# twesterhout/distributed-matvec

Hardware: AMD Instinct MI355X
Metric: matvecs/sec (higher is better)
Workload: dtype f64; 1 GPU; heisenberg_chain_32: y <- H x, 601080390 basis states, 9927521280 off-diagonal non-zeros, f64 vectors, sigma/x/y resident in HBM; partitions=1, partitioning=single, exchange=none, kernel=direct-pull+staged, x=u(hash(sigma, 42)) - 0.5, exchange_bytes_per_matvec=0

## Files before the change

### distributed-matvec_amd/_lib.py

```python
from __future__ import annotations

import ctypes as C
import os

_HERE = os.path.dirname(os.path.abspath(__file__))
LIB_PATH = os.path.join(_HERE, os.environ.get("LS_AMD_LIB", "libls_amd.so"))

c_u64p = C.POINTER(C.c_uint64)
c_i64p = C.POINTER(C.c_int64)
c_f64p = C.POINTER(C.c_double)
c_intp = C.POINTER(C.c_int)


class ChplExternalArray(C.Structure):

    _fields_ = [("elts", C.c_void_p), ("num_elts", C.c_uint64), ("freer", C.c_void_p)]


class LsHsBasis(C.Structure):

    _fields_ = [
        ("number_sites", C.c_int),
        ("number_particles", C.c_int),
        ("number_up", C.c_int),
# ... 72 lines not shown
        "ls_amd_device_count": (C.c_int, []),
        "ls_amd_set_device": (C.c_int, [C.c_int]),
        "ls_amd_malloc": (C.c_int, [C.POINTER(vp), C.c_size_t]),
        "ls_amd_free": (C.c_int, [vp]),
        "ls_amd_memcpy_h2d": (C.c_int, [vp, vp, C.c_size_t]),
        "ls_amd_memcpy_d2h": (C.c_int, [vp, vp, C.c_size_t]),
        "ls_amd_memcpy_d2d": (C.c_int, [vp, vp, C.c_size_t, vp]),
        "ls_amd_memset": (C.c_int, [vp, C.c_int, C.c_size_t, vp]),
        "ls_amd_synchronize": (C.c_int, [vp]),
        "ls_amd_stream_copy": (C.c_int, [vp, vp, C.c_int64, vp]),
        "ls_amd_stream_read": (C.c_int, [vp, C.c_int64, C.c_int, vp, vp]),
        "ls_amd_orth_max_rows": (C.c_int, []),
        "ls_amd_orth_pass": (C.c_int, [C.c_int, C.c_int64, vp, C.c_int64, vp, vp, vp, vp]),
        "ls_amd_basis_rotate": (C.c_int, [C.c_int, C.c_int, C.c_int64, vp, C.c_int64, vp, vp]),
        "ls_amd_orth_block_max_rows": (C.c_int, []),
        "ls_amd_orth_block_pass": (C.c_int, [C.c_int, C.c_int, C.c_int64, vp, C.c_int64, vp, C.c_int64, vp, vp, vp]),
        "ls_amd_block_rotate": (C.c_int, [C.c_int, C.c_int, C.c_int64, vp, C.c_int64, vp, vp]),
        "ls_amd_pointer_kind": (C.c_int, [vp]),
        "ls_amd_host_register": (C.c_int, [vp, C.c_size_t]),
        "ls_amd_host_unregister": (C.c_int, [vp]),
        "ls_amd_boundary_stats_get": (None, [C.POINTER(BoundaryStats), C.c_int]),
        "ls_amd_hash64_01": (C.c_uint64, [C.c_uint64]),
        "ls_amd_locale_idx_of": (C.c_int, [C.c_uint64, C.c_int]),
        "ls_amd_plan_create": (C.c_int, [C.POINTER(vp), op, C.c_int, C.c_int, C.c_int, C.POINTER(vp), c_i64p, C.c_int, C.c_int, vp]),
        "ls_amd_plan_create_replicated": (C.c_int, [C.POINTER(vp), op, C.c_int, C.c_int, C.c_int, vp, C.c_int64, vp, C.c_int64, vp]),
        "ls_amd_matvec_replicated": (C.c_int, [vp, vp, vp, vp]),
        "ls_amd_plan_destroy": (None, [vp]),
        "ls_amd_plan_num_rounds": (C.c_int, [vp]),
        "ls_amd_plan_kernel_name": (C.c_char_p, [vp]),
        "ls_amd_plan_send_counts": (C.c_int, [vp, C.c_int, c_i64p]),
        "ls_amd_plan_packet_bytes": (C.c_int, [vp]),
        "ls_amd_plan_row_bytes": (C.c_int, [vp]),
        "ls_amd_plan_nnz": (C.c_int64, [vp]),
        "ls_amd_plan_cache_slots": (C.c_int64, [vp, C.c_int64]),
        "ls_amd_plan_slot_cache_rows": (C.c_int, [vp, C.POINTER(C.c_int64), C.POINTER(C.c_int64)]),
        "ls_amd_matvec": (C.c_int, [vp, C.POINTER(vp), C.POINTER(vp), vp]),
        "ls_amd_matvec_block": (C.c_int, [vp, C.c_int, vp, C.c_int64, C.c_int64, vp, C.c_int64, C.c_int64, vp]),
        "ls_amd_plan_block_kernel_name": (C.c_char_p, [vp, C.c_int]),
        "ls_amd_matvec_block_axpby": (C.c_int, [vp, C.c_int, vp, C.c_int64, C.c_int64, vp, C.c_int64, C.c_int64, C.c_double, C.c_double,
                                                C.c_double, vp, vp]),
        "ls_amd_plan_axpby_kernel_name": (C.c_char_p, [vp, C.c_int]),
        "ls_amd_block_axpby_dots": (C.c_int, [C.c_int, C.c_int64, C.c_int, vp, C.c_int64, C.c_int64, vp, C.c_int64, C.c_int64, vp, C.c_int64,
                                              C.c_int64, C.c_double, C.c_double, C.c_double, vp, vp]),
        "ls_amd_matvec_block_axpby_acc": (C.c_int, [vp, C.c_int, vp, C.c_int64, C.c_int64, vp, C.c_int64, C.c_int64, C.c_double, C.c_double,
                                                    C.c_double, vp, C.c_int64, C.c_int64, C.c_int, C.c_double, C.c_double, vp, vp]),
        "ls_amd_plan_acc_kernel_name": (C.c_char_p, [vp, C.c_int]),
        "ls_amd_block_axpby_acc": (C.c_int, [C.c_int, C.c_int, C.c_int64, C.c_int, vp, C.c_int64, C.c_int64, vp, C.c_int64, C.c_int64, vp,
                                             C.c_int64, C.c_int64, vp, C.c_int64, C.c_int64, C.c_double, C.c_double, C.c_double, C.c_double,
                                             C.c_double, vp, vp]),
        "ls_amd_matvec_block_series": (C.c_int, [vp, C.c_int, C.c_int, vp, C.c_double, C.c_double, vp, C.c_int64, C.c_int64, vp, C.c_int64,
                                                 C.c_int64, C.c_int, vp, vp]),
        "ls_amd_plan_series_kernel_name": (C.c_char_p, [vp, C.c_int]),
        "ls_amd_plan_check": (C.c_int, [vp, vp]),
        "ls_amd_plan_enable_timing": (C.c_int, [vp, C.c_int]),
        "ls_amd_plan_kernel_times": (C.c_int, [vp, C.POINTER(C.c_float), C.c_int, c_intp]),
        "ls_amd_plan_enable_stage_timing": (C.c_int, [vp, C.c_int]),
        "ls_amd_plan_stage_times": (C.c_int, [vp, c_f64p, c_i64p, c_i64p]),
        "ls_amd_plan_timing_report": (C.c_int, [vp, C.c_char_p, C.c_size_t]),
        "ls_amd_operator_adjoint": (op, [op]),
        "ls_amd_operator_maps_sector": (C.c_int, [op, bp]),
        "ls_amd_operator_maps_sector_signed": (C.c_int, [op, bp]),
        "ls_amd_cross_create": (C.c_int, [C.POINTER(vp), op, bp, C.c_int, vp, C.c_int64, vp, C.c_int64, vp]),
        "ls_amd_operator_maps_subgroup_sector": (C.c_int, [op, bp]),
        "ls_amd_cross_create_groups": (C.c_int, [C.POINTER(vp), op, bp, C.c_int, C.c_int, vp, C.c_int64, vp, C.c_int64, vp]),
        "ls_amd_cross_apply": (C.c_int, [vp, vp, vp, vp]),
        "ls_amd_cross_apply_block": (C.c_int, [vp, C.c_int, vp, C.c_int64, C.c_int64, vp, C.c_int64, C.c_int64, vp]),
# ... 212 lines not shown
```

### distributed-matvec_amd/api.py

```python
from __future__ import annotations

import ctypes as C
from dataclasses import dataclass

import numpy as np

from . import _lib
from . import config as _config
from ._lib import LsAmdError

__all__ = [
    "Basis", "Operator", "LsAmdError", "loadConfigFromYaml", "loadConfigFromDict", "enumerateStates",
    "arrFromBlockToHashed", "arrFromHashedToBlock", "matrixVectorProduct", "localMatrixVector",
    "localeIdxOf", "hash64_01", "MatvecPlan", "ReplicatedPlan", "build_library", "fillRandom",
    "Communicator", "DistMatvec", "ReplMatvec", "block_axpby_dots", "block_axpby_acc", "CrossSectorPlan",
    "CsrMatrix",
]


def build_library(verbose: bool = False):
    import os
    import subprocess

    csrc = os.path.join(os.path.dirname(os.path.abspath(__file__)), "csrc")
# ... 461 lines not shown
        self.reps = reps
        self.P = num_partitions if num_partitions is not None else len(reps)
        self.me = my_partition
        self.cplx = dtype in (torch.complex128, "c128")
        n = len(reps)
        ptrs = (C.c_void_p * n)(*[r.data_ptr() for r in reps])
        counts = (C.c_int64 * n)(*[r.numel() for r in reps])
        h = C.c_void_p()
        _lib.check(L.ls_amd_plan_create(C.byref(h), matrix.payload, 1 if self.cplx else 0, self.P, my_partition,
                                        ptrs, counts, num_rounds, self.MODES[mode], _stream_ptr()))
        self.h = h

    def destroy(self):
        if getattr(self, "h", None):
            _lib.load().ls_amd_plan_destroy(self.h)
            self.h = None

    def __del__(self):
        try:
            self.destroy()
        except Exception:
            pass

    @property
    def kernel(self): return _lib.load().ls_amd_plan_kernel_name(self.h).decode()
    @property
    def num_rounds(self): return int(_lib.load().ls_amd_plan_num_rounds(self.h))
    @property
    def nnz(self): return int(_lib.load().ls_amd_plan_nnz(self.h))
    @property
    def packet_bytes(self): return int(_lib.load().ls_amd_plan_packet_bytes(self.h))
    @property
    def row_bytes(self): return int(_lib.load().ls_amd_plan_row_bytes(self.h))
    @property
    def key_bytes(self):
        return int(_lib.load().ls_amd_plan_key_bytes(self.h))
    @property
    def packet_index_bytes(self): return int(_lib.load().ls_amd_plan_packet_index_bytes(self.h))

    def segment_bytes(self, count: int) -> int:
        return int(_lib.load().ls_amd_plan_segment_bytes(self.h, int(count)))

    def segment_value_offset(self, count: int) -> int:
        return int(_lib.load().ls_amd_plan_segment_value_offset(self.h, int(count)))

    def cache_slots(self, max_bytes: int = 0) -> int:
        rows = int(_lib.load().ls_amd_plan_cache_slots(self.h, int(max_bytes)))
        if rows < 0:
            _lib.check(-1)
        return rows

    @property
    def slot_cache(self):
        r, b = C.c_int64(0), C.c_int64(0)
        _lib.load().ls_amd_plan_slot_cache_rows(self.h, C.byref(r), C.byref(b))
        return int(r.value), int(b.value)

    def send_counts(self, rnd: int):
        c = (C.c_int64 * self.P)()
        _lib.check(_lib.load().ls_amd_plan_send_counts(self.h, rnd, c))
        return [int(v) for v in c]

    def matvec(self, x, y, check: bool = True):
        xs = (C.c_void_p * len(x))(*[t.data_ptr() for t in x])
        ys = (C.c_void_p * len(y))(*[t.data_ptr() for t in y])
        _lib.check(_lib.load().ls_amd_matvec(self.h, xs, ys, _stream_ptr()))
# ... 535 lines not shown
```

### distributed-matvec_amd/csrc/host.c

```c
#define _GNU_SOURCE
#include <math.h>
#include <pthread.h>
#include <stdarg.h>
#include <stdio.h>
#include <stdlib.h>
#include <string.h>

#include "../../include/ls_amd.h"
#include "../../include/ls_chpl.h"
#include "../../include/ls_hs.h"
#include "lsk.h"

static __thread char g_last_error[1024] = "";
static ls_amd_error_handler g_handler = NULL;

static int set_error(char const *fmt, ...) {
    va_list ap;
    va_start(ap, fmt);
    vsnprintf(g_last_error, sizeof(g_last_error), fmt, ap);
    va_end(ap);
    return -1;
}
static int dev_error(void) { return set_error("%s", lsk_last_error()); }
int ls_amd_internal_error(char const *fmt, ...) {
// ... 1545 lines not shown
    int *d_err;
    int64_t nnz;
    lsk_gdir gd;
    lsk_rankdir *d_gdir;
    lsk_part_ctx *d_part_ctx;
    int part_ctx_any;
    int key_bytes;
    int streams, st_S, st_tile_rows, st_wpb, st_rounds;
    int stream_gkeys;
    void **d_send_parts;
    lsk_wsrc *d_wsrcs;
    lsk_index gindex;
    uint32_t *d_gtable;
    int64_t *d_row_gidx;
    double *d_norms_global;
    lsk_tilemap tilemap;
    void *d_tilemap;
    int has_pairs;
    int has_push_staged;
    int one_rank_full_basis;
    lsk_pairplan pairs;
    void *d_pair_recs, *d_rank_low, *d_pair_binom, *d_states32, *d_pair_rows, *d_pair_sites;
    int global_index;
    int has_hubbard;
    lsk_hubbard hubbard;
    void *d_hub[6];
    int has_chain;
    int chain_cached;
    void *d_chain_cache;
    int chain_wide;
    uint64_t *d_chain_rec;
    void *d_chain_wave;
    int chain_row_bytes;
    double chain_v[2];
    int64_t chain_row0;
    void *d_htab;
    uint32_t *d_slot_of;
    int htab_bits;
    void *d_xs;
    int pull_halo;
    int idx_mode;
    struct ls_amd_gtab *gtab;
    uint64_t *d_vtab;
    int64_t row_g0;
    lsk_pullbuf pbuf;
    int64_t split_rows;
    int64_t split_active;
    int slot_cache, slot_cache_valid;
    int64_t slot_cache_bytes;
    lsk_pullbuf blk_pbuf;
    int64_t blk_rows;
    lsk_tilemap blk_tilemap;
    void *d_blk_tilemap;
    void *d_blk_cols;
    void *d_series_work;
    int series_cols;
    double *d_series_dots;
    void const *y_checked[2];
    int leaves_basis;
    int t_capacity, t_count;
    void **t_start, **t_stop;
    int st_capacity, st_count;
    void **st_start, **st_stop;
    unsigned char *st_stage;
    double st_ms[8];
    int64_t st_calls[8];
// ... 523 lines not shown
    int const L = NBITS(op->basis);
    int const inv = op->basis->spin_inversion != 0;
    if (inv && (pl->dbs.proj != LSK_PROJ_INVERSION || pl->family != FAMILY_DIRECT_PULL || (L & 1) || BEXT(op->basis)->hamming_weight != L / 2)) return 0;
    if (L > 64 || (!inv && pl->dbs.proj != LSK_PROJ_NONE) ||
        !ext->is_real || !ext->is_hermitian || ext->runs.n_runs <= 0 || ext->n_diag <= 0)
        return 0;
    int extra = 0;
    if (inv) for (int q = 0; q < ext->runs.n_runs; ++q) if (ext->runs.lo0[q] + ext->runs.cnt[q] - 1 == L - 2) extra = 1;
    if (ext->n_groups - ext->runs.n_run_groups + extra > 2) return 0;
    for (int g = ext->runs.n_run_groups; g < ext->n_groups; ++g) {
        lsk_group const *G = &ext->groups[g];
        if (G->fast != LSK_GROUP_EXCHANGE || G->v_im != 0.0 || __builtin_popcountll(G->x) != 2) return 0;
    }
    return 1;
}
static void chain_wave_tables(int low_site, uint16_t *U, uint16_t *Rg, int *class_off) {
    int pos[13];
    uint16_t rank_in[4096];
    memset(class_off, 0, sizeof(int) * 14);
    for (int w = 0; w < 4096; ++w) ++class_off[__builtin_popcount(w) + 1];
    for (int k = 0; k < 13; ++k) { class_off[k + 1] += class_off[k]; pos[k] = class_off[k]; }
    for (int w = 0; w < 4096; ++w) {
        int const k = __builtin_popcount(w);
        rank_in[w] = (uint16_t)(pos[k] - class_off[k]);
        U[pos[k]++] = (uint16_t)w;
    }
    for (int w = 0; w < 4096; ++w) Rg[w] = low_site >= 0 ? rank_in[w ^ (1 << low_site)] : 0;
}
int ls_amd_test_chain_wave_tables(int low_site, uint16_t *U, uint16_t *Rg, int *class_off) {
    if (low_site >= 12) return set_error("ls_amd_test_chain_wave_tables: the low site lies below bit 12");
    chain_wave_tables(low_site, U, Rg, class_off);
    return 0;
}
static int setup_chain_headers(ls_amd_plan *pl, lsk_index index, int64_t n, uint64_t const *d_reps, int nc, uint64_t xmask, void *stream) {
    int const L = NBITS(pl->op->basis);
    char const *e = getenv("LS_AMD_CHAIN_RECORDS");
    int headed = !(e && atoi(e) != 0) && L >= 13 && L <= 32 && pl->dbs.proj == LSK_PROJ_NONE && pl->chain_row0 == 0 &&
                 pl->family == FAMILY_DIRECT_PULL && pl->dbs.hamming_weight >= 0 && nc <= 1;
    int lo = -1, hi = -1;
    if (headed && nc == 1) {
        lo = __builtin_ctzll(xmask);
        hi = 63 - __builtin_clzll(xmask);
        if (lo >= 12 || hi < 12) { headed = 0; lo = hi = -1; }
    }
    int const words = lsk_chain_words();
    int64_t const n_hdr = (n + 63) / 64;
    uint16_t U[4096], Rg[4096];
    int class_off[14];
    uint32_t *tab = (uint32_t *)malloc(sizeof(uint32_t) * (size_t)words);
    if (!tab) return set_error("out of memory");
    chain_wave_tables(headed ? lo : -1, U, Rg, class_off);
    for (int t = 0; t < words; ++t) tab[t] = (uint32_t)U[t] | ((uint32_t)Rg[U[t]] << 16) | (lo >= 0 ? (((uint32_t)U[t] >> lo) & 1u) << 31 : 0u);
    size_t const tab_bytes = sizeof(uint32_t) * (size_t)words, hdr_bytes = 8 * (size_t)n_hdr;
    void *q;
    if (lsk_malloc(&q, tab_bytes + hdr_bytes + 8) != 0) { free(tab); return 1; }
    unsigned long long plain = 0;
    unsigned long long *d_plain = (unsigned long long *)((char *)q + tab_bytes + hdr_bytes);
    int const rc = lsk_h2d(q, tab, tab_bytes) || lsk_h2d(d_plain, &plain, 8) ||
                   lsk_chain_headers(pl->dbs, index, n, d_reps, headed, hi, (char *)q + tab_bytes, d_plain, stream) || lsk_sync(stream) ||
                   lsk_d2h(&plain, d_plain, 8);
    free(tab);
    if (rc) { lsk_free(q); return dev_error(); }
    pl->d_chain_wave = q;
    int const rec = pl->cplx ? 4 + 4 * nc : 8;
    pl->chain_row_bytes = headed ? (int)((8 * (uint64_t)n_hdr + 64 * (uint64_t)rec * (uint64_t)plain + (uint64_t)n - 1) / (uint64_t)n) : rec;
    return 0;
}
static int setup_chain(ls_amd_plan *pl, lsk_index index, int64_t n, uint64_t const *d_reps, void *stream) {
    struct ls_amd_operator_ext const *ext = OEXT(pl->op);
    int nc = ext->n_groups - ext->runs.n_run_groups;
    int const Ls = NBITS(pl->op->basis);
    int const inv = pl->dbs.proj == LSK_PROJ_INVERSION;
    uint64_t const top = 1ULL << (Ls - 1);
    uint64_t cx[3];
    double cv[3];
    int k = 0;
    if (inv)
        for (int q = 0; q < pl->dop.runs.n_runs; ++q)
            if (pl->dop.runs.lo0[q] + pl->dop.runs.cnt[q] - 1 == Ls - 2) {
                cx[k] = 3ULL << (Ls - 2);
                cv[k++] = pl->dop.runs.v_re[q] * (double)pl->op->basis->spin_inversion;
                if (--pl->dop.runs.cnt[q] == 0) {
                    for (int r = q; r + 1 < pl->dop.runs.n_runs; ++r) {
                        pl->dop.runs.lo0[r] = pl->dop.runs.lo0[r + 1]; pl->dop.runs.cnt[r] = pl->dop.runs.cnt[r + 1];
                        pl->dop.runs.v_re[r] = pl->dop.runs.v_re[r + 1]; pl->dop.runs.v_im[r] = pl->dop.runs.v_im[r + 1];
                    }
                    --pl->dop.runs.n_runs;
                }
                break;
            }
    for (int g = ext->runs.n_run_groups; g < ext->n_groups && k < 3; ++g) {
        cx[k] = ext->groups[g].x;
        cv[k++] = ext->groups[g].v_re * ((inv && (ext->groups[g].x & top)) ? (double)pl->op->basis->spin_inversion : 1.0);
    }
    nc = k;
    if (nc > 2) return 0;
    char const *ew = getenv("LS_AMD_CHAIN_WIDE");
    pl->chain_wide = index.count >= 0xffffffffLL || (ew && atoi(ew) != 0 && NBITS(pl->op->basis) > 32);
    size_t const es = pl->chain_wide ? sizeof(uint64_t) : sizeof(uint32_t);
    if (nc > 0 && n > 0) {
        void *q;
        if (lsk_malloc(&q, es * (size_t)nc * (size_t)n) != 0) return 0;
        pl->d_chain_cache = q;
        int zero = 0, flag = 0;
        DEV(lsk_h2d(pl->d_err, &zero, sizeof(int)));
        for (int c = 0; c < nc; ++c)
            DEV(lsk_chain_cache(pl->dbs, index, n, d_reps, cx[c],
                                (char *)pl->d_chain_cache + es * (size_t)c * (size_t)n, pl->chain_wide, pl->d_err, stream));
        DEV(lsk_sync(stream));
        DEV(lsk_d2h(&flag, pl->d_err, sizeof(int)));
        DEV(lsk_h2d(pl->d_err, &zero, sizeof(int)));
        if (flag) {
            lsk_free(pl->d_chain_cache);
            pl->d_chain_cache = NULL;
            return 0;
        }
        pl->chain_cached = nc;
        pl->chain_v[0] = cv[0];
        pl->chain_v[1] = nc > 1 ? cv[1] : 0.0;
    }
    if (build_tilemap(pl, n, lsk_chain_tile_rows(pl->cplx)) != 0) return -1;
    if (!pl->cplx && NBITS(pl->op->basis) <= 32 && !pl->chain_wide && n > 0) {
        void *q;
        if (lsk_malloc(&q, sizeof(uint64_t) * (size_t)n) != 0) {
            if (pl->d_chain_cache) { lsk_free(pl->d_chain_cache); pl->d_chain_cache = NULL; }
            if (pl->d_tilemap) { lsk_free(pl->d_tilemap); pl->d_tilemap = NULL; memset(&pl->tilemap, 0, sizeof(pl->tilemap)); }
            pl->chain_cached = 0;
            return 0;
        }
        pl->d_chain_rec = (uint64_t *)q;
        DEV(lsk_chain_pack(n, d_reps, pl->chain_cached ? pl->d_chain_cache : NULL, (uint64_t *)q, stream));
        DEV(lsk_sync(stream));
        if (pl->chain_cached <= 1 && pl->d_chain_cache) { lsk_free(pl->d_chain_cache); pl->d_chain_cache = NULL; }
    }
    if (NBITS(pl->op->basis) <= 32 && !pl->chain_wide && n > 0) {
        int const rc = setup_chain_headers(pl, index, n, d_reps, pl->chain_cached, pl->chain_cached > 0 ? cx[0] : 0, stream);
        if (rc < 0) return -1;
        if (rc > 0) {
            if (pl->d_chain_rec) { lsk_free(pl->d_chain_rec); pl->d_chain_rec = NULL; }
            if (pl->d_chain_cache) { lsk_free(pl->d_chain_cache); pl->d_chain_cache = NULL; }
            if (pl->d_tilemap) { lsk_free(pl->d_tilemap); pl->d_tilemap = NULL; memset(&pl->tilemap, 0, sizeof(pl->tilemap)); }
            pl->chain_cached = 0;
            return 0;
        }
    }
    pl->has_chain = 1;
    return 0;
}

static int pair_cmp(void const *pa, void const *pb) {
    lsk_pair const *a = (lsk_pair const *)pa, *b = (lsk_pair const *)pb;
    int const ca = a->j < 11 ? 0 : (a->i < 11 ? 1 : 2), cb = b->j < 11 ? 0 : (b->i < 11 ? 1 : 2);
    if (ca != cb) return ca - cb;
    if (a->i != b->i) return (int)a->i - (int)b->i;
    return (int)a->j - (int)b->j;
}
static int setup_pairs(ls_amd_plan *pl, int64_t n, uint64_t const *d_reps, void *stream) {
    ls_hs_operator const *op = pl->op;
    struct ls_amd_operator_ext const *ext = OEXT(op);
    int const L = NBITS(op->basis), hw = BEXT(op->basis)->hamming_weight;
    char const *e = getenv("LS_AMD_ROW_KERNEL");
    if (e && strcmp(e, "generic") == 0) return 0;
    int const wide = L > 32;
    if (L > 64 || hw < 0 || hw + 2 > LSK_PAIR_KC || op->basis->spin_inversion != 0 || pl->dbs.proj != LSK_PROJ_NONE || !ext->is_real ||
        !ext->is_hermitian || ext->n_groups < 1 || ext->n_groups > LSK_MAX_PAIRS || n <= 0 || n >= 0xffffffffLL ||
        ext->n_diag <= 0)
        return 0;
    int const force_sites = e && strcmp(e, "pairsites") == 0;
    int const by_row = force_sites || (e && strcmp(e, "pairrows") == 0) || (!(e && strcmp(e, "pairs") == 0) && (11 * hw < 4 * L || 11 * (L - hw) < 4 * L));
    lsk_pair recs[LSK_MAX_PAIRS];
    memset(recs, 0, sizeof(recs));
// ... 1084 lines not shown
                              pl->gindex.count, d_x_global, pl->pull_halo, d_y_local, pl->d_err, stream));
    stage_end(pl, st, stream);
    return 0;
}
int ls_amd_internal_repl_split_finish(ls_amd_plan *pl, void const *d_x_global, void *d_y_local, void *stream) {
    if (pl->family != FAMILY_REPL_TILE || !pl->idx_mode || pl->split_rows <= 0) return ls_amd_matvec_replicated(pl, d_x_global, d_y_local, stream);
    return ls_amd_internal_repl_split_rows(pl, d_x_global, d_y_local, 0, pl->parts[0].count, 1, stream);
}
char const *ls_amd_plan_kernel_name(ls_amd_plan const *pl) {
    switch (pl->family) {
    case FAMILY_DIRECT_PUSH: return pl->has_push_staged ? "direct-push+staged" : "direct-push";
    case FAMILY_DIRECT_PULL:
        if (pl->has_hubbard) return "direct-pull+hubbard";
        return pl->has_chain ? "direct-pull+staged" : pl->has_pairs ? (pl->pairs.sites ? "direct-pull+pairsites" : pl->pairs.rows ? "direct-pull+pairrows" : "direct-pull+pairs") : "direct-pull";
    case FAMILY_TILE_PULL: return pl->idx_mode ? (pl->slot_cache ? "tile-pull+indexed+cached" : (pl->d_vtab ? "tile-pull+values" : "tile-pull+indexed")) : "tile-pull";
    case FAMILY_REPL_DIRECT:
        return pl->has_chain ? "replicated-direct-pull+staged" : "replicated-direct-pull";
    case FAMILY_REPL_TILE: return pl->idx_mode ? (pl->slot_cache ? "replicated-tile-pull+indexed+cached" : "replicated-tile-pull+indexed") : "replicated-tile-pull";
    default: return pl->streams ? "tile+streams" : (pl->has_push_staged ? "tile(one rank: push+staged)" : "tile");
    }
}
int ls_amd_plan_packet_bytes(ls_amd_plan const *pl) { return pl->key_bytes + (pl->cplx ? 16 : 8); }
int ls_amd_plan_row_bytes(ls_amd_plan const *pl) {
    if (pl->has_hubbard) return 0;
    if (pl->has_pairs) return pl->pairs.wide ? 8 : 4;
    if (pl->has_chain) {
        if (pl->d_chain_wave) return pl->chain_row_bytes;
        int const narrow = NBITS(pl->op->basis) <= 32 && !pl->chain_wide;
        return (narrow ? 4 : 8) + pl->chain_cached * (pl->chain_wide ? 8 : 4);
    }
    if (pl->family == FAMILY_TILE_PULL || pl->family == FAMILY_REPL_TILE) return 16;
    return 8;
}
int64_t ls_amd_plan_nnz(ls_amd_plan const *pl) { return pl->nnz; }
int ls_amd_plan_send_counts(ls_amd_plan const *pl, int round, int64_t *counts) {
    if (pl->family != FAMILY_TILE) { for (int d = 0; d < pl->P; ++d) counts[d] = 0; return 0; }
    part_state const *ps = &pl->parts[0];
    if (round < 0 || round >= ps->rounds) return set_error("round out of range");
    memcpy(counts, ps->send_counts + (size_t)round * pl->P, sizeof(int64_t) * pl->P);
    return 0;
}

static int prescaled_x(ls_amd_plan *pl, int64_t n, uint64_t const *d_reps, void const *d_x, double const *d_norms,
                       void const **out, void *stream) {
    if (!pl->d_htab) {
        int bits = 4;
        while (((int64_t)1 << bits) < 2 * n) ++bits;
        if (bits > 32) return set_error("hash index: more than 2^31 representatives per table are not supported");
        pl->htab_bits = bits;
        DEV(lsk_malloc(&pl->d_htab, (size_t)(pl->cplx ? 32 : 16) << bits));
        void *p;
        DEV(lsk_malloc(&p, 4 * (size_t)(n > 0 ? n : 1)));
        pl->d_slot_of = (uint32_t *)p;
        DEV(lsk_hash_build(pl->cplx, n, d_reps, bits, pl->d_htab, pl->d_slot_of, stream));
        pl->pull_halo = pull_halo_setting(0);
        if (pl->pull_halo > 0 && pl->dbs.k4_mode != 0) DEV(lsk_malloc(&pl->d_xs, (size_t)(pl->cplx ? 16 : 8) * (size_t)(n > 0 ? n : 1)));
    }
    int const st = stage_begin(pl, ST_REFRESH, stream);
    DEV(lsk_hash_fill(pl->cplx, n, pl->d_slot_of, d_x, pl->dbs.k4_mode != 0 ? d_norms : NULL, pl->d_htab, pl->d_xs, stream));
    stage_end(pl, st, stream);
    *out = pl->d_htab;
    return 0;
}

int ls_amd_diag(ls_amd_plan *pl, void const *d_x, void *d_y, void *stream) {
    part_state *ps = &pl->parts[0];
// ... 3324 lines not shown
```

### distributed-matvec_amd/csrc/k_rows.hip

```cpp
#include <hip/hip_runtime.h>
#include "lsk_dev.hpp"

template <bool CPLX>
__global__ __launch_bounds__(kBlock) void k_diag(lsk_runs runs, int n_diag, lsk_term const *__restrict__ diag,
                                                 int64_t n, uint64_t const *__restrict__ reps,
                                                 double const *__restrict__ x, double *__restrict__ y) {
    for (int64_t i = (int64_t)blockIdx.x * kBlock + threadIdx.x; i < n; i += (int64_t)gridDim.x * kBlock) {
        uint64_t a = reps[i];
        double dr, di;
        diag_coeff<uint64_t, false>(runs, n_diag, diag, a, dr, di);
        if (CPLX) {
            double xr = x[2 * i], xi = x[2 * i + 1];
            y[2 * i] = dr * xr - di * xi;
            y[2 * i + 1] = dr * xi + di * xr;
        } else {
            y[i] = dr * x[i];
        }
    }
}

extern "C" int lsk_diag(lsk_operator op, int cplx, int64_t n, uint64_t const *reps, void const *x, void *y,
                        void *stream) {
    if (n == 0 || op.n_diag == 0) return 0;
    dim3 g(grid_for(n)), b(kBlock);
// ... 559 lines not shown
    constexpr int LDSP = CPLX ? 11 : kChainLdsPairs;
    constexpr int WINDOW = TILE + 2 * HALO + 2;
    constexpr int FAR = CPLX ? kChainFarC : kChainFar;
    constexpr R kNone = ~(R)0;
    constexpr int hb = kChainLdsPairs;
    X const *__restrict__ x = (X const *)x_v;
    X *__restrict__ y = (X *)y_v;
    const bool extra_stream = kAblate && (n_cached & 0x100);
    const int nt_from = !kAblate ? 99 : ((n_cached & 0x200) ? 20 : ((n_cached & 0x400) ? 0 : 99));
    if (kAblate) n_cached &= 0xff;
    uint64_t ex_next = 0;
    extern __shared__ uint4 s_img[];
    R const *const s_binom = reinterpret_cast<R const *>(s_img);
    uint2 const *const s_near = reinterpret_cast<uint2 const *>(reinterpret_cast<char const *>(s_img) + near_off);
    __shared__ X s_x[WINDOW + 1];
    for (int k = threadIdx.x; k < img16; k += kBlock) s_img[k] = g_img[k];
    (void)NB;
    if (threadIdx.x == 0) s_x[WINDOW] = cx_zero<X>();
    const int xcd = blockIdx.x & 7;
    const int64_t blocks_per_xcd = gridDim.x >> 3;
    const int lane = threadIdx.x & 63;
    tilemap += (int64_t)xcd * slots_per_xcd;
    uint32_t const *__restrict__ reps32 = reinterpret_cast<uint32_t const *>(reps);
    constexpr bool HDR = REC || (CPLX && sizeof(W) == 4 && sizeof(R) == 4);
    constexpr int NSUB = TILE / kBlock;
    for (int64_t t = blockIdx.x >> 3; t < slots_per_xcd; t += blocks_per_xcd) {
        const uint64_t slot = tilemap[t];
        const int cnt = (int)(slot >> 48);
        if (cnt == 0) continue;
        const int64_t i0 = (int64_t)(slot & 0xffffffffffffULL);
        const int64_t w0 = (row0 + i0 - HALO) & ~(int64_t)1;
        W a_next = 0;
        R t0_next = kNone, t1_next = kNone;
        auto load_row = [&](int64_t row, W &a_out, R &t0_out, R &t1_out) {
            if (REC) {
                const uint64_t rec = __builtin_nontemporal_load(reps + row);
                a_out = (W)(uint32_t)rec;
                t0_out = (R)(uint32_t)(rec >> 32);
            } else {
                if (sizeof(W) == 4) a_out = (W)__builtin_nontemporal_load(reps32 + 2 * row);
                else a_out = (W)__builtin_nontemporal_load(reps + row);
                if (n_cached > 0) t0_out = __builtin_nontemporal_load(cache + row);
            }
            if (n_cached > 1) t1_out = __builtin_nontemporal_load(cache + (size_t)n + (size_t)row);
            if (kAblate && extra_stream) ex_next = __builtin_nontemporal_load(reps + (row < (n >> 1) ? row + (n >> 1) : row - (n >> 1)));
        };
        const int wave0 = (int)(threadIdx.x & ~63u);
        uint32_t hq = ~0u;
        if (HDR) {
            const uint32_t hw = 2 * (uint32_t)(i0 >> 6) + 2 * ((threadIdx.x >> 6) + (uint32_t)(lane % NSUB) * (kBlock / 64)) + (lane / NSUB) % 2;
            if (((int64_t)(hw >> 1) << 6) < n) hq = wave_plan[kChainWords + hw];
        }
        auto fetch_row = [&](int s, int64_t row) {
            if (HDR) {
                const uint32_t ti = (uint32_t)__builtin_amdgcn_readlane((int)hq, s) & (kChainWords - 1u);
                if (ti != kChainWords - 1u) { a_next = (W)wave_plan[ti + lane]; return; }
            }
            load_row(row, a_next, t0_next, t1_next);
        };
        if (wave0 < cnt) {
            const int64_t rr = i0 + ((int)threadIdx.x < cnt ? (int)threadIdx.x : cnt - 1);
            fetch_row(0, rr);
        }
        __syncthreads();
        if (CPLX) {
            for (int j = threadIdx.x; j < WINDOW; j += kBlock) {
                const int64_t row = w0 + j;
                s_x[j] = (row >= 0 && row < n_x) ? x[row] : cx_zero<X>();
            }
        } else {
            double const *xd = (double const *)x_v;
            double *sd = (double *)s_x;
            for (int j = 2 * threadIdx.x; j < WINDOW; j += 2 * kBlock) {
                const int64_t row = w0 + j;
                double2 v;
                if (row >= 0 && row + 1 < n_x) v = *reinterpret_cast<double2 const *>(xd + row);
                else { v.x = (row >= 0 && row < n_x) ? xd[row] : 0.0; v.y = (row + 1 >= 0 && row + 1 < n_x) ? xd[row + 1] : 0.0; }
                sd[j] = v.x;
                sd[j + 1] = v.y;
            }
        }
        __syncthreads();
        const int own0 = (int)(row0 + i0 - w0);
        X y_pending = cx_zero<X>();
        int r_pending = -1;
#pragma unroll 1
        for (int sub = 0; sub < TILE / kBlock; ++sub) {
            const int r = sub * kBlock + threadIdx.x;
            if (r_pending >= 0) cx_store_nt(y + i0 + r_pending, y_pending);
            r_pending = -1;
            W a = a_next;
// ... 187 lines not shown
                                                       uint32_t const *__restrict__ cache, uint64_t *__restrict__ out) {
    for (int64_t i = (int64_t)blockIdx.x * kBlock + threadIdx.x; i < n; i += (int64_t)gridDim.x * kBlock)
        out[i] = (uint64_t)(uint32_t)reps[i] | ((uint64_t)(cache ? cache[i] : 0xffffffffu) << 32);
}
extern "C" int lsk_chain_pack(int64_t n, uint64_t const *reps, void const *cache, uint64_t *out, void *stream) {
    if (n == 0) return 0;
    hipLaunchKernelGGL(k_chain_pack, dim3(grid_for(n)), dim3(kBlock), 0, (hipStream_t)stream, n, reps, (uint32_t const *)cache, out);
    LSK_LAUNCH_CHECK();
    return 0;
}

__global__ __launch_bounds__(kBlock) void k_chain_headers(int64_t n, uint64_t const *__restrict__ reps, int hamming_weight, int high_site,
                                                          uint64_t const *__restrict__ g_binom, uint2 *__restrict__ out,
                                                          unsigned long long *__restrict__ n_plain) {
    const int64_t n_hdr = (n + 63) >> 6;
    for (int64_t w = (int64_t)blockIdx.x * kBlock + threadIdx.x; w < n_hdr; w += (int64_t)gridDim.x * kBlock) {
        uint2 h = make_uint2(~0u, ~0u);
        const uint32_t first = (uint32_t)reps[w << 6];
        if ((w << 6) + 63 < n && ((first ^ (uint32_t)reps[(w << 6) + 63]) >> 12) == 0) {
            const uint32_t high = first & ~(kChainWords - 1u), low = first & (kChainWords - 1u);
            const int kl = __popc(low);
            uint32_t ti = (uint32_t)rank_combinadic_w<uint32_t, uint64_t>(low, g_binom);
            for (int k = 0; k < kl; ++k) ti += (uint32_t)g_binom[12 * LSK_BINOM_K + k];
            uint32_t base = 0;
            if (high_site >= 0) {
                const uint32_t hbit = (high >> high_site) & 1u;
                const int kp = hbit ? kl + 1 : kl - 1;
                if (kp >= 0 && kp <= 12 && kp <= hamming_weight)
                    base = (uint32_t)rank_combinadic_w<uint32_t, uint64_t>((high ^ (1u << high_site)) | ((1u << kp) - 1u), g_binom);
                base |= hbit << 31;
            }
            h = make_uint2(high | ti, base);
        } else
            atomicAdd(n_plain, 1ULL);
        out[w] = h;
    }
}
extern "C" int lsk_chain_headers(lsk_basis bs, lsk_index ix, int64_t n, uint64_t const *reps, int headed, int high_site, void *out,
                                 unsigned long long *d_n_plain, void *stream) {
    if (n == 0) return 0;
    if (!headed) {
        if (hipMemsetAsync(out, 0xff, 8 * (size_t)((n + 63) >> 6), (hipStream_t)stream) != hipSuccess) { snprintf(g_err, sizeof(g_err), "lsk_chain_headers: memset failed"); return -1; }
        return 0;
    }
    if (bs.number_sites > 32 || bs.number_sites < 13 || bs.hamming_weight < 0 || high_site >= bs.number_sites || (high_site >= 0 && high_site < 12)) {
        snprintf(g_err, sizeof(g_err), "lsk_chain_headers: plan out of range");
        return -1;
    }
    hipLaunchKernelGGL(k_chain_headers, dim3(grid_for((n + 63) >> 6)), dim3(kBlock), 0, (hipStream_t)stream, n, reps, bs.hamming_weight,
                       high_site, ix.binom, (uint2 *)out, d_n_plain);
    LSK_LAUNCH_CHECK();
    return 0;
}
extern "C" int lsk_chain_words(void) { return (int)kChainWords; }

__global__ void k_binom_narrow(uint64_t const *__restrict__ in, uint32_t *__restrict__ out, int n) {
    for (int k = blockIdx.x * blockDim.x + threadIdx.x; k < n; k += gridDim.x * blockDim.x) out[k] = (uint32_t)in[k];
}
template <typename R> static R const *chain_binom(uint64_t const *g_binom, hipStream_t stream);
template <> uint64_t const *chain_binom<uint64_t>(uint64_t const *g_binom, hipStream_t) { return g_binom; }
template <> uint32_t const *chain_binom<uint32_t>(uint64_t const *g_binom, hipStream_t stream) {
    static uint64_t const *src = nullptr;
    static uint32_t *narrow = nullptr;
    static std::mutex lock;
    std::lock_guard<std::mutex> guard(lock);
    if (src != g_binom || !narrow) {
        if (!narrow && hipMalloc((void **)&narrow, sizeof(uint32_t) * 64 * LSK_BINOM_K) != hipSuccess) return nullptr;
        hipLaunchKernelGGL(k_binom_narrow, dim3(4), dim3(kBlock), 0, stream, g_binom, narrow, 64 * LSK_BINOM_K);
        src = g_binom;
    }
    return narrow;
}

static int chain_near_fill(uint64_t const (*C)[LSK_BINOM_K], int elem, int ldsp, int16_t *near) {
    int const base[3] = {0, 32, 192};
    for (int g = 0; g < 3; ++g)
        for (int kidx = 0; kidx <= 4 * g; ++kidx)
            for (int pat = 0; pat < 32; ++pat)
                for (int p = 0; p < 4; ++p) {
                    int const lo = 4 * g + p;
                    int const bit = (pat >> p) & 1, nxt = (pat >> (p + 1)) & 1;
                    int const k = kidx + __builtin_popcount(pat & ((1 << p) - 1));
                    int64_t const d = (int64_t)C[lo][k < LSK_BINOM_K ? k : 0] * elem;
// ... 551 lines not shown
```

### distributed-matvec_amd/csrc/lsk.h

```cpp
#ifndef LSK_H
#define LSK_H

#include <stddef.h>
#include <stdint.h>

#ifdef __cplusplus
extern "C" {
#endif

#define LSK_BENES_STAGES 11
#define LSK_BINOM_K 34
#define LSK_MAX_PARTS 256

typedef struct lsk_term {
    double v_re, v_im;
    uint64_t m, r, s;
} lsk_term;

enum { LSK_GROUP_GENERIC = 0, LSK_GROUP_EXCHANGE = 1,
       LSK_GROUP_HOP_LO = 2, LSK_GROUP_HOP_HI = 3 };

typedef struct lsk_group {
    uint64_t x;
    double v_re, v_im;
// ... 181 lines not shown
    lsk_pair const *pairs;
    uint16_t const *rank_low;
    uint32_t const *binom;
    void const *states;
    int wide;
    double dsum;
    lsk_pair_row const *rows;
    uint32_t const *sites;
    int n_sites, degree;
    int n_classes, site_words;
} lsk_pairplan;
int lsk_push_tile_rows(int cplx);
int lsk_push_staged(lsk_operator op, lsk_basis bs, lsk_index ix, int cplx, lsk_tilemap tm, int64_t n, uint64_t const *reps,
                    void const *x, void *y, int *d_err, void *stream);
int lsk_pairs_tile_rows(int cplx);
int lsk_pairs(lsk_pairplan pp, int hamming_weight, int cplx, lsk_tilemap tm, int64_t n, void const *x, void *y, void *stream);
typedef struct lsk_species {
    int64_t n;
    int deg;
    uint32_t const *words;
    uint32_t const *rank;
    double const *coef;
} lsk_species;
typedef struct lsk_hubbard {
    int L, cplx_coef;
    lsk_species up, dn;
} lsk_hubbard;
int lsk_hubbard_apply(lsk_hubbard hb, lsk_operator op, int cplx, lsk_tilemap tm, void const *x, void *y, void *stream);
int lsk_narrow_states(int64_t n, uint64_t const *reps, uint32_t *out, void *stream);

int lsk_chain_pack(int64_t n, uint64_t const *reps, void const *cache, uint64_t *out, void *stream);
int lsk_chain_headers(lsk_basis bs, lsk_index ix, int64_t n, uint64_t const *reps, int headed, int high_site, void *out,
                      unsigned long long *d_n_plain, void *stream);
int lsk_chain_words(void);
int lsk_chain_cache(lsk_basis bs, lsk_index ix, int64_t n, uint64_t const *reps, uint64_t xmask, void *out, int wide_ranks,
                    int *d_flag, void *stream);
int lsk_tile(lsk_operator op, lsk_basis bs, lsk_index ix, int cplx, int count_only, int P, int me,
             int64_t row0, int64_t row1, uint64_t const *reps, double const *norms, void const *x,
             void *y, unsigned long long *d_cursors, lsk_round_layout const *d_layout, void *d_send,
             unsigned long long *d_counts, int *d_err, void *stream);
int lsk_tile_wv_max_parts(void);
int lsk_tile_wv(lsk_operator op, lsk_basis bs, lsk_index ix, lsk_gdir gd, int cplx, int count_only, int P, int me,
                int64_t row0, int64_t row1, uint64_t const *reps, double const *norms, void const *x, void *y,
                uint32_t *d_wtab, lsk_round_layout const *d_layout, void *d_send, int *d_err, lsk_gtab own_gt, void *stream);
int lsk_tile_st_max_classes(void);
int lsk_tile_st(lsk_operator op, lsk_gdir gd, uint64_t const *d_binom, int cplx, int count_only, int P, int S, int tile_rows,
                int64_t row0, int64_t row1, uint64_t const *reps, void const *x, uint32_t *d_ttab,
                lsk_round_layout const *d_layout, void *d_send, int *d_err, void *stream);
typedef struct lsk_wsrc {
    uint32_t const *keys;
    double const *vals;
    uint32_t const *soff;
} lsk_wsrc;
typedef struct lsk_wdests {
    int n;
    int64_t count[LSK_MAX_SEGS];
    int64_t first_block[LSK_MAX_SEGS + 1];
    void *y[LSK_MAX_SEGS];
    lsk_rankdir const *dir[LSK_MAX_SEGS];
    uint64_t const *reps[LSK_MAX_SEGS];
    uint64_t const *binom;
    int64_t n_ranks;
    int weight;
    int *err;
} lsk_wdests;
int lsk_window_rows(int cplx);
// ... 308 lines not shown
```

### include/ls_amd.h

```cpp
#ifndef LS_AMD_H
#define LS_AMD_H

#include "ls_hs.h"

#ifdef __cplusplus
extern "C" {
#endif

typedef enum { LS_AMD_F64 = 0, LS_AMD_C128 = 1 } ls_amd_dtype;

typedef enum {
    LS_AMD_MODE_AUTO = 0,
    LS_AMD_MODE_PUSH = 1,
    LS_AMD_MODE_PULL = 2
} ls_amd_mode;

typedef struct ls_amd_plan ls_amd_plan;

char const *ls_amd_last_error(void);
typedef void (*ls_amd_error_handler)(char const *message);
void ls_amd_set_error_handler(ls_amd_error_handler handler);

int ls_amd_device_count(void);
int ls_amd_set_device(int device);
// ... 59 lines not shown
int ls_amd_dist_matvec(ls_amd_dist *dist, void const *d_x, void *d_y, void *stream);
ls_amd_plan *ls_amd_dist_plan(ls_amd_dist *dist);
int64_t ls_amd_dist_exchange_bytes(ls_amd_dist const *dist);
int ls_amd_dist_num_rounds(ls_amd_dist const *dist);

typedef struct ls_amd_repl ls_amd_repl;
int ls_amd_repl_create(ls_amd_repl **repl, ls_amd_comm *comm, ls_hs_operator const *op, ls_amd_dtype dtype,
                       uint64_t const *d_reps_global, uint8_t const *d_masks, int64_t count_global, void *stream);
void ls_amd_repl_destroy(ls_amd_repl *repl);
int ls_amd_repl_matvec(ls_amd_repl *repl, void const *d_x_local, void *d_y_local, void *stream);
ls_amd_plan *ls_amd_repl_plan(ls_amd_repl *repl);
int64_t ls_amd_repl_exchange_bytes(ls_amd_repl const *repl);
int64_t ls_amd_repl_x_in_bytes(ls_amd_repl const *repl);
int ls_amd_test_corrupt_dist(ls_amd_dist *dist);
void ls_amd_test_set_stream_windows_per_block(int n);
void ls_amd_test_fail_stream_buffers(int on);
void ls_amd_test_fail_dist_streams(int on);
int ls_amd_test_corrupt_repl(ls_amd_repl *repl);
int ls_amd_comm_wait(ls_amd_comm *comm, void *stream, double timeout_s);
void ls_amd_test_skew_exchange(int rank, int64_t delta_bytes, int late);
int ls_amd_comm_test_stall(ls_amd_comm *comm, double seconds);
int ls_amd_test_corrupt_plan(ls_amd_plan *plan);

int ls_amd_plan_create(ls_amd_plan **plan, ls_hs_operator const *op, ls_amd_dtype dtype,
                       int num_partitions, int my_partition, uint64_t const *const *d_reps,
                       int64_t const *counts, int num_rounds, ls_amd_mode mode, void *stream);
void ls_amd_plan_destroy(ls_amd_plan *plan);

int ls_amd_plan_num_rounds(ls_amd_plan const *plan);
char const *ls_amd_plan_kernel_name(ls_amd_plan const *plan);
int ls_amd_plan_send_counts(ls_amd_plan const *plan, int round, int64_t *counts);
int ls_amd_plan_packet_bytes(ls_amd_plan const *plan);
int ls_amd_plan_row_bytes(ls_amd_plan const *plan);
int64_t ls_amd_plan_nnz(ls_amd_plan const *plan);

int64_t ls_amd_plan_cache_slots(ls_amd_plan *plan, int64_t max_bytes);
int ls_amd_plan_slot_cache_rows(ls_amd_plan const *plan, int64_t *rows, int64_t *bytes);

int ls_amd_matvec(ls_amd_plan *plan, void const *const *d_x, void *const *d_y, void *stream);

int ls_amd_matvec_block(ls_amd_plan *plan, int K, void const *d_x, int64_t x_row, int64_t x_col,
                        void *d_y, int64_t y_row, int64_t y_col, void *stream);
char const *ls_amd_plan_block_kernel_name(ls_amd_plan const *plan, int K);

int ls_amd_matvec_block_axpby(ls_amd_plan *plan, int K, void const *d_x, int64_t x_row, int64_t x_col,
                              void *d_y, int64_t y_row, int64_t y_col, double alpha, double beta, double gamma,
                              double *d_dots, void *stream);
char const *ls_amd_plan_axpby_kernel_name(ls_amd_plan const *plan, int K);
int ls_amd_block_axpby_dots(int cplx, int64_t n, int K, void const *d_w, int64_t w_row, int64_t w_col, void const *d_x, int64_t x_row,
                            int64_t x_col, void *d_y, int64_t y_row, int64_t y_col, double alpha, double beta, double gamma,
                            double *d_dots, void *stream);
int ls_amd_matvec_block_axpby_acc(ls_amd_plan *plan, int K, void const *d_x, int64_t x_row, int64_t x_col,
                                  void *d_y, int64_t y_row, int64_t y_col, double alpha, double beta, double gamma,
                                  void *d_z, int64_t z_row, int64_t z_col, int z_cplx, double c_re, double c_im,
                                  double *d_dots, void *stream);
char const *ls_amd_plan_acc_kernel_name(ls_amd_plan const *plan, int K);
int ls_amd_block_axpby_acc(int cplx, int z_cplx, int64_t n, int K, void const *d_w, int64_t w_row, int64_t w_col, void const *d_x,
                           int64_t x_row, int64_t x_col, void *d_y, int64_t y_row, int64_t y_col, void *d_z, int64_t z_row,
                           int64_t z_col, double alpha, double beta, double gamma, double c_re, double c_im, double *d_dots,
                           void *stream);
int ls_amd_matvec_block_series(ls_amd_plan *plan, int K, int N, double const *coeffs, double lo, double hi,
                               void const *d_x, int64_t x_row, int64_t x_col, void *d_z, int64_t z_row, int64_t z_col, int z_cplx,
                               void *d_work, void *stream);
char const *ls_amd_plan_series_kernel_name(ls_amd_plan const *plan, int K);
int ls_amd_plan_check(ls_amd_plan *plan, void *stream);

// ... 158 lines not shown
```

Before: 142.1 matvecs/s.

## Store chain records only for plain header blocks in compacted pages

When chain headers are active, per-row records or caches are no longer allocated for all n rows. They are allocated only for 64-row blocks that the header marks as plain (non-patterned), and those blocks are compacted into pages indexed by an atomic counter stored in the header. The pull kernel redirects loads through the page number read from the header lane. This cuts the resident chain-record footprint and the record stream traffic for rows already served by wave tables. In exchange it adds a page-build pass at plan time and an extra readlane plus index computation per row fetch.

```diff
diff --git a/distributed-matvec_amd/_lib.py b/distributed-matvec_amd/_lib.py
--- a/distributed-matvec_amd/_lib.py
+++ b/distributed-matvec_amd/_lib.py
@@ -128,6 +128,7 @@
         "ls_amd_plan_packet_bytes": (C.c_int, [vp]),
         "ls_amd_plan_row_bytes": (C.c_int, [vp]),
         "ls_amd_plan_nnz": (C.c_int64, [vp]),
+        "ls_amd_plan_chain_bytes": (C.c_int64, [vp]),
         "ls_amd_plan_cache_slots": (C.c_int64, [vp, C.c_int64]),
         "ls_amd_plan_slot_cache_rows": (C.c_int, [vp, C.POINTER(C.c_int64), C.POINTER(C.c_int64)]),
         "ls_amd_matvec": (C.c_int, [vp, C.POINTER(vp), C.POINTER(vp), vp]),
diff --git a/distributed-matvec_amd/api.py b/distributed-matvec_amd/api.py
--- a/distributed-matvec_amd/api.py
+++ b/distributed-matvec_amd/api.py
@@ -517,6 +517,9 @@
     def packet_bytes(self): return int(_lib.load().ls_amd_plan_packet_bytes(self.h))
     @property
     def row_bytes(self): return int(_lib.load().ls_amd_plan_row_bytes(self.h))
+    @property
+    def chain_bytes(self):
+        return int(_lib.load().ls_amd_plan_chain_bytes(self.h))
     @property
     def key_bytes(self):
         return int(_lib.load().ls_amd_plan_key_bytes(self.h))
diff --git a/distributed-matvec_amd/csrc/host.c b/distributed-matvec_amd/csrc/host.c
--- a/distributed-matvec_amd/csrc/host.c
+++ b/distributed-matvec_amd/csrc/host.c
@@ -1601,6 +1601,7 @@
     uint64_t *d_chain_rec;
     void *d_chain_wave;
     int chain_row_bytes;
+    int64_t chain_bytes;
     double chain_v[2];
     int64_t chain_row0;
     void *d_htab;
@@ -2190,17 +2191,24 @@
     chain_wave_tables(low_site, U, Rg, class_off);
     return 0;
 }
-static int setup_chain_headers(ls_amd_plan *pl, lsk_index index, int64_t n, uint64_t const *d_reps, int nc, uint64_t xmask, void *stream) {
+static int chain_headers_serve(ls_amd_plan const *pl, int64_t n, int nc, uint64_t xmask, int *lo, int *hi) {
     int const L = NBITS(pl->op->basis);
     char const *e = getenv("LS_AMD_CHAIN_RECORDS");
-    int headed = !(e && atoi(e) != 0) && L >= 13 && L <= 32 && pl->dbs.proj == LSK_PROJ_NONE && pl->chain_row0 == 0 &&
-                 pl->family == FAMILY_DIRECT_PULL && pl->dbs.hamming_weight >= 0 && nc <= 1;
-    int lo = -1, hi = -1;
-    if (headed && nc == 1) {
-        lo = __builtin_ctzll(xmask);
-        hi = 63 - __builtin_clzll(xmask);
-        if (lo >= 12 || hi < 12) { headed = 0; lo = hi = -1; }
-    }
+    *lo = *hi = -1;
+    if ((e && atoi(e) != 0) || L < 13 || L > 32 || pl->chain_wide || n <= 0 || pl->dbs.proj != LSK_PROJ_NONE || pl->chain_row0 != 0 ||
+        pl->family != FAMILY_DIRECT_PULL || pl->dbs.hamming_weight < 0 || nc > 1)
+        return 0;
+    if (nc == 1) {
+        int const l = __builtin_ctzll(xmask), h = 63 - __builtin_clzll(xmask);
+        if (l >= 12 || h < 12) return 0;
+        *lo = l;
+        *hi = h;
+    }
+    return 1;
+}
+static int setup_chain_headers(ls_amd_plan *pl, lsk_index index, int64_t n, uint64_t const *d_reps, int nc, uint64_t xmask, void *stream) {
+    int lo, hi;
+    int const headed = chain_headers_serve(pl, n, nc, xmask, &lo, &hi);
     int const words = lsk_chain_words();
     int64_t const n_hdr = (n + 63) / 64;
     uint16_t U[4096], Rg[4096];
@@ -2220,6 +2228,23 @@
     free(tab);
     if (rc) { lsk_free(q); return dev_error(); }
     pl->d_chain_wave = q;
+    pl->chain_bytes += (int64_t)(tab_bytes + hdr_bytes + 8);
+    if (headed) {
+        size_t const slot = pl->cplx ? sizeof(uint32_t) : sizeof(uint64_t), bytes = slot * 64 * (size_t)(plain > 0 ? plain : 1);
+        void *pg = NULL;
+        int zero = 0, flag = 0;
+        if (!pl->cplx || nc > 0) {
+            if (lsk_malloc(&pg, bytes) != 0) return 1;
+            if (pl->cplx) pl->d_chain_cache = pg; else pl->d_chain_rec = (uint64_t *)pg;
+            pl->chain_bytes += (int64_t)bytes;
+        }
+        if (pg && (lsk_memset_async(pg, 0xff, bytes, stream) || lsk_h2d(pl->d_err, &zero, sizeof(int)) ||
+                   lsk_chain_pages(pl->dbs, index, n, d_reps, (char *)q + tab_bytes, nc > 0 ? xmask : 0, pl->cplx ? NULL : (uint64_t *)pg,
+                                   pl->cplx ? pg : NULL, pl->d_err, stream) ||
+                   lsk_sync(stream) || lsk_d2h(&flag, pl->d_err, sizeof(int)) || lsk_h2d(pl->d_err, &zero, sizeof(int))))
+            return dev_error();
+        if (flag) return 1;
+    }
     int const rec = pl->cplx ? 4 + 4 * nc : 8;
     pl->chain_row_bytes = headed ? (int)((8 * (uint64_t)n_hdr + 64 * (uint64_t)rec * (uint64_t)plain + (uint64_t)n - 1) / (uint64_t)n) : rec;
     return 0;
@@ -2256,10 +2281,18 @@
     char const *ew = getenv("LS_AMD_CHAIN_WIDE");
     pl->chain_wide = index.count >= 0xffffffffLL || (ew && atoi(ew) != 0 && NBITS(pl->op->basis) > 32);
     size_t const es = pl->chain_wide ? sizeof(uint64_t) : sizeof(uint32_t);
-    if (nc > 0 && n > 0) {
+    int lo_site, hi_site;
+    int const paged = chain_headers_serve(pl, n, nc, nc > 0 ? cx[0] : 0, &lo_site, &hi_site);
+    if (paged && nc > 0) {
+        pl->chain_cached = nc;
+        pl->chain_v[0] = cv[0];
+        pl->chain_v[1] = 0.0;
+    }
+    if (nc > 0 && n > 0 && !paged) {
         void *q;
         if (lsk_malloc(&q, es * (size_t)nc * (size_t)n) != 0) return 0;
         pl->d_chain_cache = q;
+        pl->chain_bytes += (int64_t)(es * (size_t)nc * (size_t)n);
         int zero = 0, flag = 0;
         DEV(lsk_h2d(pl->d_err, &zero, sizeof(int)));
         for (int c = 0; c < nc; ++c)
@@ -2271,6 +2304,7 @@
         if (flag) {
             lsk_free(pl->d_chain_cache);
             pl->d_chain_cache = NULL;
+            pl->chain_bytes = 0;
             return 0;
         }
         pl->chain_cached = nc;
@@ -2278,23 +2312,27 @@
         pl->chain_v[1] = nc > 1 ? cv[1] : 0.0;
     }
     if (build_tilemap(pl, n, lsk_chain_tile_rows(pl->cplx)) != 0) return -1;
-    if (!pl->cplx && NBITS(pl->op->basis) <= 32 && !pl->chain_wide && n > 0) {
+    if (!pl->cplx && NBITS(pl->op->basis) <= 32 && !pl->chain_wide && n > 0 && !paged) {
         void *q;
         if (lsk_malloc(&q, sizeof(uint64_t) * (size_t)n) != 0) {
             if (pl->d_chain_cache) { lsk_free(pl->d_chain_cache); pl->d_chain_cache = NULL; }
             if (pl->d_tilemap) { lsk_free(pl->d_tilemap); pl->d_tilemap = NULL; memset(&pl->tilemap, 0, sizeof(pl->tilemap)); }
             pl->chain_cached = 0;
+            pl->chain_bytes = 0;
             return 0;
         }
         pl->d_chain_rec = (uint64_t *)q;
+        pl->chain_bytes += (int64_t)(sizeof(uint64_t) * (size_t)n);
         DEV(lsk_chain_pack(n, d_reps, pl->chain_cached ? pl->d_chain_cache : NULL, (uint64_t *)q, stream));
         DEV(lsk_sync(stream));
-        if (pl->chain_cached <= 1 && pl->d_chain_cache) { lsk_free(pl->d_chain_cache); pl->d_chain_cache = NULL; }
+        if (pl->chain_cached <= 1 && pl->d_chain_cache) { lsk_free(pl->d_chain_cache); pl->d_chain_cache = NULL; pl->chain_bytes -= (int64_t)(es * (size_t)n); }
     }
     if (NBITS(pl->op->basis) <= 32 && !pl->chain_wide && n > 0) {
         int const rc = setup_chain_headers(pl, index, n, d_reps, pl->chain_cached, pl->chain_cached > 0 ? cx[0] : 0, stream);
         if (rc < 0) return -1;
         if (rc > 0) {
+            if (pl->d_chain_wave) { lsk_free(pl->d_chain_wave); pl->d_chain_wave = NULL; }
+            pl->chain_bytes = 0;
             if (pl->d_chain_rec) { lsk_free(pl->d_chain_rec); pl->d_chain_rec = NULL; }
             if (pl->d_chain_cache) { lsk_free(pl->d_chain_cache); pl->d_chain_cache = NULL; }
             if (pl->d_tilemap) { lsk_free(pl->d_tilemap); pl->d_tilemap = NULL; memset(&pl->tilemap, 0, sizeof(pl->tilemap)); }
@@ -3445,6 +3483,7 @@
     if (pl->family == FAMILY_TILE_PULL || pl->family == FAMILY_REPL_TILE) return 16;
     return 8;
 }
+int64_t ls_amd_plan_chain_bytes(ls_amd_plan const *pl) { return pl->has_chain ? pl->chain_bytes : 0; }
 int64_t ls_amd_plan_nnz(ls_amd_plan const *pl) { return pl->nnz; }
 int ls_amd_plan_send_counts(ls_amd_plan const *pl, int round, int64_t *counts) {
     if (pl->family != FAMILY_TILE) { for (int d = 0; d < pl->P; ++d) counts[d] = 0; return 0; }
diff --git a/distributed-matvec_amd/csrc/k_rows.hip b/distributed-matvec_amd/csrc/k_rows.hip
--- a/distributed-matvec_amd/csrc/k_rows.hip
+++ b/distributed-matvec_amd/csrc/k_rows.hip
@@ -615,15 +615,15 @@
         const int64_t w0 = (row0 + i0 - HALO) & ~(int64_t)1;
         W a_next = 0;
         R t0_next = kNone, t1_next = kNone;
-        auto load_row = [&](int64_t row, W &a_out, R &t0_out, R &t1_out) {
+        auto load_row = [&](int64_t row, int64_t prow, W &a_out, R &t0_out, R &t1_out) {
             if (REC) {
-                const uint64_t rec = __builtin_nontemporal_load(reps + row);
+                const uint64_t rec = __builtin_nontemporal_load(reps + prow);
                 a_out = (W)(uint32_t)rec;
                 t0_out = (R)(uint32_t)(rec >> 32);
             } else {
                 if (sizeof(W) == 4) a_out = (W)__builtin_nontemporal_load(reps32 + 2 * row);
                 else a_out = (W)__builtin_nontemporal_load(reps + row);
-                if (n_cached > 0) t0_out = __builtin_nontemporal_load(cache + row);
+                if (n_cached > 0) t0_out = __builtin_nontemporal_load(cache + prow);
             }
             if (n_cached > 1) t1_out = __builtin_nontemporal_load(cache + (size_t)n + (size_t)row);
             if (kAblate && extra_stream) ex_next = __builtin_nontemporal_load(reps + (row < (n >> 1) ? row + (n >> 1) : row - (n >> 1)));
@@ -635,11 +635,14 @@
             if (((int64_t)(hw >> 1) << 6) < n) hq = wave_plan[kChainWords + hw];
         }
         auto fetch_row = [&](int s, int64_t row) {
+            int64_t prow = row;
             if (HDR) {
                 const uint32_t ti = (uint32_t)__builtin_amdgcn_readlane((int)hq, s) & (kChainWords - 1u);
                 if (ti != kChainWords - 1u) { a_next = (W)wave_plan[ti + lane]; return; }
-            }
-            load_row(row, a_next, t0_next, t1_next);
+                const uint32_t page = (uint32_t)__builtin_amdgcn_readlane((int)hq, NSUB + s);
+                if (page != ~0u) prow = (int64_t)((page << 6) | ((uint32_t)row & 63u));
+            }
+            load_row(row, prow, a_next, t0_next, t1_next);
         };
         if (wave0 < cnt) {
             const int64_t rr = i0 + ((int)threadIdx.x < cnt ? (int)threadIdx.x : cnt - 1);
@@ -893,7 +896,7 @@
             }
             h = make_uint2(high | ti, base);
         } else
-            atomicAdd(n_plain, 1ULL);
+            h.y = (uint32_t)atomicAdd(n_plain, 1ULL);
         out[w] = h;
     }
 }
@@ -910,6 +913,36 @@
     }
     hipLaunchKernelGGL(k_chain_headers, dim3(grid_for((n + 63) >> 6)), dim3(kBlock), 0, (hipStream_t)stream, n, reps, bs.hamming_weight,
                        high_site, ix.binom, (uint2 *)out, d_n_plain);
+    LSK_LAUNCH_CHECK();
+    return 0;
+}
+__global__ __launch_bounds__(kBlock) void k_chain_pages(int64_t n, uint64_t const *__restrict__ reps, uint2 const *__restrict__ headers, uint64_t xmask,
+                                                        int hamming_weight, uint64_t const *__restrict__ g_binom, uint64_t *__restrict__ rec,
+                                                        uint32_t *__restrict__ cache, int *__restrict__ flag) {
+    __shared__ uint32_t s_binom[32 * LSK_BINOM_K];
+    for (int k = threadIdx.x; k < 32 * LSK_BINOM_K; k += blockDim.x) s_binom[k] = (uint32_t)g_binom[k];
+    __syncthreads();
+    for (int64_t i = (int64_t)blockIdx.x * kBlock + threadIdx.x; i < n; i += (int64_t)gridDim.x * kBlock) {
+        const uint2 h = headers[i >> 6];
+        if ((h.x & (kChainWords - 1u)) != kChainWords - 1u) continue;
+        const uint32_t a = (uint32_t)reps[i];
+        uint32_t t = ~0u;
+        if (__popc(a & (uint32_t)xmask) == 1) {
+            const uint32_t beta = a ^ (uint32_t)xmask;
+            if (__popc(beta) != hamming_weight) atomicExch(flag, 1);
+            else t = (uint32_t)rank_combinadic_w<uint32_t, uint32_t>(beta, s_binom);
+        }
+        const size_t slot = ((size_t)h.y << 6) + (size_t)(i & 63);
+        if (rec) rec[slot] = (uint64_t)a | ((uint64_t)t << 32);
+        if (cache) cache[slot] = t;
+    }
+}
+extern "C" int lsk_chain_pages(lsk_basis bs, lsk_index ix, int64_t n, uint64_t const *reps, void const *headers, uint64_t xmask, uint64_t *rec,
+                               void *cache, int *d_flag, void *stream) {
+    if (n == 0 || (!rec && !cache)) return 0;
+    if (bs.number_sites > 32 || bs.hamming_weight < 0 || bs.proj != LSK_PROJ_NONE) { snprintf(g_err, sizeof(g_err), "lsk_chain_pages: plan out of range"); return -1; }
+    hipLaunchKernelGGL(k_chain_pages, dim3(grid_for(n)), dim3(kBlock), 0, (hipStream_t)stream, n, reps, (uint2 const *)headers, xmask,
+                       bs.hamming_weight, ix.binom, rec, (uint32_t *)cache, d_flag);
     LSK_LAUNCH_CHECK();
     return 0;
 }
diff --git a/distributed-matvec_amd/csrc/lsk.h b/distributed-matvec_amd/csrc/lsk.h
--- a/distributed-matvec_amd/csrc/lsk.h
+++ b/distributed-matvec_amd/csrc/lsk.h
@@ -237,6 +237,8 @@
 int lsk_chain_pack(int64_t n, uint64_t const *reps, void const *cache, uint64_t *out, void *stream);
 int lsk_chain_headers(lsk_basis bs, lsk_index ix, int64_t n, uint64_t const *reps, int headed, int high_site, void *out,
                       unsigned long long *d_n_plain, void *stream);
+int lsk_chain_pages(lsk_basis bs, lsk_index ix, int64_t n, uint64_t const *reps, void const *headers, uint64_t xmask, uint64_t *rec,
+                    void *cache, int *d_flag, void *stream);
 int lsk_chain_words(void);
 int lsk_chain_cache(lsk_basis bs, lsk_index ix, int64_t n, uint64_t const *reps, uint64_t xmask, void *out, int wide_ranks,
                     int *d_flag, void *stream);
diff --git a/include/ls_amd.h b/include/ls_amd.h
--- a/include/ls_amd.h
+++ b/include/ls_amd.h
@@ -115,6 +115,7 @@
 int ls_amd_plan_send_counts(ls_amd_plan const *plan, int round, int64_t *counts);
 int ls_amd_plan_packet_bytes(ls_amd_plan const *plan);
 int ls_amd_plan_row_bytes(ls_amd_plan const *plan);
+int64_t ls_amd_plan_chain_bytes(ls_amd_plan const *plan);
 int64_t ls_amd_plan_nnz(ls_amd_plan const *plan);
 
 int64_t ls_amd_plan_cache_slots(ls_amd_plan *plan, int64_t max_bytes);
```

Result: no change. 141.8 matvecs/s (-0.2%).
